# EtherealEngine/Universal-Volumetric

Hardware: AMD Instinct MI355X
Metric: frames/s encode, 100k-vert mesh + 2048^2 texture (higher is better)
Workload: dtype u8/int32 (f32 only in the quantiser)

## Files before the change

universal-volumetric_amd/csrc/geo_conn.hpp:

```cpp
__global__ void __launch_bounds__(UVOL_BLOCK) k_face_time(GeoJob *jobs) {
  JOB_OR_RETURN;
  const uint32_t i = blockIdx.x * UVOL_BLOCK + threadIdx.x;
  if (i < (uint32_t)J.nsym) { const int c = J.proc[i]; J.face_time[c / 3] = (int32_t)i; J.tstart[J.nsym - 1 - (int)i] = code_of_corner(c); }
  if (i < (uint32_t)J.ninit) { const int c = J.initc[i]; J.face_time[c / 3] = -(int32_t)i - 2; J.tstart[J.nsym + (int)i] = code_of_corner(c); }
}
__device__ __forceinline__ int att_vertex(const GeoJob &J, int slot, int c);
__device__ __forceinline__ int rec_vertex_field(const GeoJob &J, int t, int c, int r8) {
  if (r8 == 2) { const uint32_t *q = reinterpret_cast<const uint32_t *>(J.rec[1 + t]) + 4 * (size_t)(c / 3); return (int)((uint32_t)((((uint64_t)q[1] << 32) | q[0]) >> (21 * (c % 3))) & 0x1fffffu); }
  const size_t code = (size_t)code_of_corner(c);
  return r8 ? (int)((uint32_t)J.rec[1 + t][2 * code] & 0x1fffffu) : J.rec[1 + t][4 * code];
}
__global__ void __launch_bounds__(UVOL_BLOCK) k_v2d(GeoJob *jobs, int r8) {
  GeoJob &J = jobs[blockIdx.y];
  const int t = blockIdx.z;
  const uint32_t i = blockIdx.x * UVOL_BLOCK + threadIdx.x;
  const bool live = J.status == 0 && !(t > 0 && (t - 1 >= J.nad || !J.interior_seams[t - 1]));
  if (blockIdx.x * UVOL_BLOCK >= (live ? J.ne[t] : 0u)) return;
  int lo0 = 0x7fffffff, hi0 = -0x7fffffff - 1, lo1 = 0x7fffffff, hi1 = -0x7fffffff - 1;
  int iu = -1;
  if (J.qpos) for (int k = 0; k < J.nad; k++) if (J.att_kind[k] == 0 && (J.interior_seams[k] ? t == 1 + k : t == 0)) iu = k;
  if (i < J.ne[t]) {
    const int c = J.order[t][i];
    int vid, pid = 0;
    if (!J.qpos) vid = rec_vertex_field(J, t, c, r8) >> 1;
// ... 32 lines not shown
__global__ void __launch_bounds__(UVOL_BLOCK) k_eb_event_flags(GeoJob *jobs) {
  JOB_OR_RETURN_UNIFORM;
  const uint32_t i = blockIdx.x * UVOL_BLOCK + threadIdx.x;
  uint32_t n = 0;
  if (i < J.nf) { int a[2], b[2]; n = i < (uint32_t)J.nsym ? (uint32_t)eb_events_of(J, i, a, b) : 0u; J.evcnt[i] = (uint8_t)n; }
  const uint32_t tot = block_sum(n);
  if (threadIdx.x == 0 && blockIdx.x < uvol_blocks_dev(J.nf)) J.bsum2[blockIdx.x] = tot;
}
__global__ void __launch_bounds__(UVOL_BLOCK) k_eb_event_compact(GeoJob *jobs) {
  GeoJob &J = jobs[blockIdx.y];
  const uint32_t i = blockIdx.x * UVOL_BLOCK + threadIdx.x;
  if (J.status == 0 && blockIdx.x != 0 && blockIdx.x < uvol_blocks_dev(J.nf) && J.bsum2[blockIdx.x + 1] == J.bsum2[blockIdx.x]) return;
  const bool live = J.status == 0 && i < J.nf;
  uint32_t v = live ? J.evcnt[i] : 0, tot;
  const uint32_t pos = block_excl_scan(v, &tot) + ((J.status == 0 && blockIdx.x <= uvol_blocks_dev(J.nf)) ? J.bsum2[blockIdx.x] : 0);
  if (live && v) {
    int a[2], b[2]; const int n = eb_events_of(J, i, a, b);
    if (pos + (uint32_t)n > J.evcap) J.status = GEO_E_WS_OVERFLOW;
    else for (int k = 0; k < n; k++) { J.ev_src[pos + k] = (int)i; J.ev_spl[pos + k] = a[k]; J.ev_edge[pos + k] = (uint8_t)b[k]; }
  }
  if (blockIdx.x == 0 && threadIdx.x == 0 && J.status == 0) J.nev = (int)J.bsum2[uvol_blocks_dev(J.nf)];
}

__global__ void __launch_bounds__(UVOL_BLOCK) k_valence_init(GeoJob *jobs) {
  JOB_OR_RETURN;
  const uint32_t t = blockIdx.x * UVOL_BLOCK + threadIdx.x, stride = gridDim.x * UVOL_BLOCK;
  { const uint32_t n4 = J.nc / 4;
    const uint4 *src = reinterpret_cast<const uint4 *>(geo_vt(J)); uint4 *dst = reinterpret_cast<uint4 *>(J.c2vm);
    for (uint32_t q = t; q < n4; q += stride) dst[q] = src[q];
    for (uint32_t c = 4 * n4 + t; c < J.nc; c += stride) J.c2vm[c] = geo_vt(J)[c]; }
  const uint32_t nv0 = J.nverts_t[0] < J.ecap ? J.nverts_t[0] : J.ecap;
  for (uint32_t v = t; v < nv0; v += stride) J.vval[v] = J.ring_d[v];
}
__global__ void __launch_bounds__(64) k_eb_valence(GeoJob *jobs) {
  GeoJob &J = jobs[blockIdx.x];
  UVOL_SERIAL_PRIO();
  const uint32_t lane = threadIdx.x;
  const bool ok = J.status == 0;
  const int nsym = ok ? J.nsym : 0, nc = (int)J.nc;
  const int32_t *opp = J.opp, *proc = J.proc, *ftime = J.face_time; const uint8_t *symb = J.symb;
  int32_t *vval = J.vval, *c2vm = J.c2vm;
  const int nv0 = ok ? (int)J.nverts_t[0] : 0;
  (void)nc;
  int nvval = nv0;
  for (int base = 0; base < nsym; base += 64) {
    const int mi = base + (int)lane;
    int c_ = 0, s_ = 0, va_ = 0, vn_ = 0, vp_ = 0;
    if (mi < nsym) { c_ = proc[mi]; s_ = symb[mi]; va_ = c2vm[c_]; vn_ = c2vm[g_nxt(c_)]; vp_ = c2vm[g_prv(c_)]; }
    const int cnt = nsym - base < 64 ? nsym - base : 64;
    const uint32_t dpk = s_ == 0 ? 0x14u : (s_ == 5 ? 0x25u : (s_ == 3 ? 0x19u : 0x2au));
    int start = 0;
    while (start < cnt) {
      const unsigned long long smask = __ballot((int)lane >= start && (int)lane < cnt && s_ == 1);
      const int e = smask ? (int)(__ffsll((long long)smask) - 1) : cnt;
      if (e > start) {
        const bool act = (int)lane >= start && (int)lane < e;
        const int v_start = act ? UVOL_ALOAD(&vval[vn_]) : 0;
        int acc = 0;
        for (int k = start; k + 1 < e; k++) {
          const int ka = (int)UVOL_READLANE(va_, k), kn = (int)UVOL_READLANE(vn_, k), kp = (int)UVOL_READLANE(vp_, k);
          const uint32_t kd = UVOL_READLANE(dpk, k);
          const int hit = (vn_ == ka ? (int)(kd & 3u) : 0) + (vn_ == kn ? (int)((kd >> 2) & 3u) : 0) + (vn_ == kp ? (int)(kd >> 4) : 0);
          acc += (int)lane > k ? hit : 0;
        }
        if (act) {
          const int av = v_start - acc;
          if (mi > 0) { const int cv = av < 2 ? 2 : (av > 7 ? 7 : av); J.ctx_of[mi] = (uint8_t)(cv - 2); }
          if (dpk & 3u) UVOL_AADD(&vval[va_], -(int)(dpk & 3u));
          UVOL_AADD(&vval[vn_], -(int)((dpk >> 2) & 3u));
          UVOL_AADD(&vval[vp_], -(int)(dpk >> 4));
        }
        UVOL_WAVE_FENCE();
        UVOL_WAVE_SYNC();
      }
      if (e < cnt) {
        const int i = base + e;
        const int lc = (int)UVOL_READLANE(c_, e);
        const int ia = (int)UVOL_READLANE(va_, e), in_ = (int)UVOL_READLANE(vn_, e), ip = (int)UVOL_READLANE(vp_, e);
        if (lane == 0) {
          const int nx = g_nxt(lc), pv = g_prv(lc);
          const int val_n = UVOL_ALOAD(&vval[in_]), val_p = UVOL_ALOAD(&vval[ip]);
          UVOL_ASTORE(&vval[in_], val_n - 1); UVOL_ASTORE(&vval[ip], val_p - 1);
          int nleft = 0, a = opp[pv];
          while (a >= 0) { if (ftime[a / 3] <= i) break; nleft++; a = opp[g_nxt(a)]; }
          UVOL_ASTORE(&vval[ia], nleft + 1);
          const int newv = nvval; int nright = 0; a = opp[nx];
          while (a >= 0) { if (ftime[a / 3] <= i) break; nright++; c2vm[g_nxt(a)] = newv; a = opp[g_prv(a)]; }
          UVOL_ASTORE(&vval[nvval], nright + 1);
          if (i > 0) { const int cv = val_n < 2 ? 2 : (val_n > 7 ? 7 : val_n); J.ctx_of[i] = (uint8_t)(cv - 2); }
        }
        nvval++;
        UVOL_WAVE_FENCE();
        UVOL_WAVE_SYNC();
        if (mi < nsym && (int)lane > e) { va_ = c2vm[c_]; vn_ = c2vm[g_nxt(c_)]; vp_ = c2vm[g_prv(c_)]; }
      }
      start = e + 1;
    }
  }
}

__global__ void __launch_bounds__(64) k_eb_ctx(GeoJob *jobs) {
  GeoJob &J = jobs[blockIdx.x];
  UVOL_SERIAL_PRIO();
  const uint32_t lane = threadIdx.x;
  const int nsym = J.status == 0 ? J.nsym : 0;
  uint32_t cnt[6] = {0, 0, 0, 0, 0, 0};
  for (int base = 1; base < nsym; base += 64) {
    const int i = base + (int)lane;
    const int cx = i < nsym ? J.ctx_of[i] : 7;
    for (int c = 0; c < 6; c++) cnt[c] += (uint32_t)__popcll(__ballot(cx == c));
  }
  uint32_t base_c[6]; { uint32_t o = 0; for (int c = 0; c < 6; c++) { base_c[c] = o; o += cnt[c]; } }
  uint32_t *all = J.ctx_all;
  const unsigned long long lt = lane == 0 ? 0ull : (~0ull >> (64 - lane));
  for (int base = 1; base < nsym; base += 64) {
    const int i = base + (int)lane;
    const bool in = i < nsym;
    const int cx = in ? J.ctx_of[i] : 7;
    const int ps = in ? J.symb[i - 1] : 0;
    const uint32_t id = ps == 0 ? 0u : (ps == 1 ? 1u : (ps == 3 ? 2u : (ps == 5 ? 3u : 4u)));
    for (int c = 0; c < 6; c++) {
      const unsigned long long m = __ballot(in && cx == c);
      if (in && cx == c) all[base_c[c] + (uint32_t)__popcll(m & lt)] = id;
      base_c[c] += (uint32_t)__popcll(m);
    }
  }
  if (lane == 0 && J.status == 0) for (int c = 0; c < 6; c++) { J.ctx_n[c] = cnt[c]; J.rs[c].n = cnt[c]; J.ctx_sym[c] = all + (base_c[c] - cnt[c]); J.rs[c].syms = J.ctx_sym[c]; }
}

__device__ __forceinline__ bool fseam_bit(const GeoJob &J, int slot, int c) { return (J.fseam[c / 3] >> (3 * slot + c % 3)) & 1u; }
__device__ __forceinline__ int st_opp(const GeoJob &J, int slot, int c) { if (c < 0) return GEO_INV; if (slot >= 0 && fseam_bit(J, slot, c)) return GEO_INV; return J.opp[c]; }
__device__ __forceinline__ int st_swl(const GeoJob &J, int slot, int c) { const int o = st_opp(J, slot, g_nxt(c)); return o < 0 ? GEO_INV : g_nxt(o); }
__device__ __forceinline__ int st_swr(const GeoJob &J, int slot, int c) { const int o = st_opp(J, slot, g_prv(c)); return o < 0 ? GEO_INV : g_prv(o); }
__device__ __forceinline__ bool vseam_bit(const GeoJob &J, int slot, uint32_t v) { return (J.vseam[slot][v >> 5] >> (v & 31)) & 1u; }
__device__ __forceinline__ int att_vertex(const GeoJob &J, int slot, int c) {
  const int v = geo_vt(J)[c];
  return (J.interior_seams[slot] && vseam_bit(J, slot, (uint32_t)v)) ? J.avert[slot][c] : v;
}
__global__ void __launch_bounds__(UVOL_BLOCK) k_seams(GeoJob *jobs) {
  JOB_OR_RETURN;
  const uint32_t f = blockIdx.x * UVOL_BLOCK + threadIdx.x;
  if (f >= J.nf) return;
  const uvol_s3 o3 = *reinterpret_cast<const uvol_s3 *>(J.opp + 3 * (size_t)f);
  const int opp_[3] = { o3.x, o3.y, o3.z };
  uint32_t bits = 0;
  for (int i = 0; i < J.nad; i++) {
    const int32_t *A = J.att_kind[i] == 0 ? J.cu : J.cn;
    const uvol_s3 a3 = *reinterpret_cast<const uvol_s3 *>(A + 3 * (size_t)f);
    const int a[3] = { a3.x, a3.y, a3.z };
    bool any = false;
    for (int k = 0; k < 3; k++) {
      uint32_t sm = 1;
      if (opp_[k] >= 0) {
        const int oo = opp_[k], fo = 3 * (oo / 3), jo = oo - fo;
        const uvol_s3 b3 = *reinterpret_cast<const uvol_s3 *>(A + fo);
        const int b[3] = { b3.x, b3.y, b3.z };
        sm = (a[(k + 1) % 3] != b[(jo + 2) % 3] || a[(k + 2) % 3] != b[(jo + 1) % 3]) ? 1u : 0u;
        if (sm) {
          any = true;
          const uint32_t va = (uint32_t)geo_vt(J)[3 * f + (k + 1) % 3], vb = (uint32_t)geo_vt(J)[3 * f + (k + 2) % 3];
// ... 94 lines not shown
```

universal-volumetric_amd/csrc/geo_walk_simt.hpp:

```cpp
#define S_REC(code, vi, rc, lc)                                                                                         \
  do {                                                                                                                  \
    if (R8) { const uvol_u2 q_ = *(UVOL_G(const uvol_u2))(rec + 2 * (size_t)(code)); rec8_dec(q_.x, q_.y, vi, rc, lc); }  \
    else { const uvol_i4 q_ = *(UVOL_G(const uvol_i4))(rec + 4 * (size_t)(code)); vi = q_.x; rc = q_.y; lc = q_.z; }      \
  } while (0)
#define S_FLAG(code) (rec[(R8 ? 2 : 4) * (size_t)((code) | 3)])
#define S_PRE(code, a, b, c, fl)                                                                                        \
  do {                                                                                                                  \
    if (R8) { const uvol_u2 q_ = *(UVOL_G(const uvol_u2))(rec + 2 * (size_t)(code)); a = q_.x; b = q_.y; c = 0; }          \
    else { const uvol_i4 q_ = *(UVOL_G(const uvol_i4))(rec + 4 * (size_t)(code)); a = (uint32_t)q_.x; b = (uint32_t)q_.y; c = (uint32_t)q_.z; } \
    fl = S_FLAG(code);                                                                                                  \
  } while (0)
#define S_TAKE(a, b, c, vi, rc, lc) do { if (R8) rec8_dec(a, b, vi, rc, lc); else { vi = (int)(a); rc = (int)(b); lc = (int)(c); } } while (0)

template <bool R8>
__device__ inline void eb_walk_simt(GeoJob &J) {
  const int nf = (int)J.nf;
  UVOL_G(uint32_t) rec = UVOL_TO_G(uint32_t, reinterpret_cast<uint32_t *>(J.rec[0]));
  UVOL_G(uint32_t) vbits = UVOL_TO_G(uint32_t, reinterpret_cast<uint32_t *>(J.vvis));
  UVOL_G(int32_t) proc = UVOL_TO_G(int32_t, J.proc); UVOL_G(int32_t) stack = UVOL_TO_G(int32_t, J.stack); UVOL_G(int32_t) initc = UVOL_TO_G(int32_t, J.initc);
  UVOL_G(uint8_t) symb = UVOL_TO_G(uint8_t, J.symb); UVOL_G(uint8_t) start_bits = UVOL_TO_G(uint8_t, J.start_bits);
  const bool rl = J.relabel != 0; UVOL_G(const int32_t) s_of_o = UVOL_TO_G(const int32_t, J.s_of_o);
  int nproc = 0, ninit = 0, nstart = 0, nsplit = 0;
  int fo = 0, sp = 0, x = -1, vi = 0, rcn = -1, lcn = -1;
  for (;;) {
// ... 412 lines not shown
      const uint32_t unf = (uint32_t)nf;
      const uint32_t rf = ((uint32_t)rcc >> 2) < unf ? ((uint32_t)rcc >> 2) : unf, lf = ((uint32_t)lcc >> 2) < unf ? ((uint32_t)lcc >> 2) : unf;
      f16_mark<FD>(rec, fc, q);
      const uvol_u4 qr = f16_load(rec, (int)rf), ql = f16_load(rec, (int)lf);
      const uint32_t v = vic >> 1;
      const uint32_t vw = vbits[v >> 5];
      const int top2 = pend_s[pend >= 2 ? pend - 2 : 0];
      vbits[v >> 5] = vw | (1u << (v & 31));
      const uint32_t vvis = (vw >> (v & 31)) & 1u;
      order[n_ord] = 3 * fc + (x & 3);
      n_ord += (int)(vvis ^ 1u);
      nvis += run ? 1 : 0;
      const uint32_t rvis = f16_seen<FD>(qr) ? 1u : 0u, lvis = f16_seen<FD>(ql) ? 1u : 0u;
      const bool ccase = ((vvis | vic) & 1u) == 0;
      const uint32_t k = ccase ? 0u : 1u + rvis + 2u * lvis;
      pend_s[pend] = lcc;
      const bool fork = k == 1u;
      if (!run) { pend--; top = top2; }
      if (fork) { pend++; top = lcc; if (pend > (int)stcap) { J.status = GEO_E_WS_OVERFLOW; done = true; } }
      if (k == 4u) { x = -1; q.x = q.z = 0; q.y = q.w = 0x80000000u; }
      else {
        const bool go_l = k == 2u;
        x = go_l ? lcc : rcc;
        q.x = go_l ? ql.x : qr.x; q.y = go_l ? ql.y : qr.y; q.z = go_l ? ql.z : qr.z; q.w = go_l ? ql.w : qr.w;
        f16_dec(q, x & 3, vi, rc, lc);
      }
    }
  }
  if (live && J.status == 0) {
    J.ne[t] = (uint32_t)n_ord;
    if (t == 0 && J.nverts != 0xffffffffu && (uint32_t)n_ord != J.nverts) J.status = -11;
  }
}
__global__ void __launch_bounds__(64) k_traverse_wave_f16(GeoJob *jobs, int n, int W, int t0, int base_hi) {
  const int t = t0 + (int)blockIdx.y;
  if (t == 0 && base_hi) traverse_wave_f16<3>(jobs, n, W, t); else traverse_wave_f16<1>(jobs, n, W, t);
}
```

universal-volumetric_amd/csrc/geom_encode.hip:

```cpp
#include <chrono>
#include <thread>
#include "uvol_common.hpp"
#include "geom_device.hpp"
#include "uvol_ws.hpp"
#include <algorithm>
#include <map>

#define JOB_OR_RETURN GeoJob &J = jobs[blockIdx.y]; if (J.status != 0) return
#define JOB_OR_RETURN_UNIFORM GeoJob &J = jobs[blockIdx.y]; { __shared__ int job_st_; if (threadIdx.x == 0) job_st_ = J.status; __syncthreads(); if (job_st_ != 0) return; }

#include "geo_scan.hpp"
#include "geo_dedup.hpp"
#include "geo_faces.hpp"
#include "geo_corner_table.hpp"
#include "geo_walk_lds.hpp"
#include "geo_conn.hpp"
#include "geo_traverse_lds.hpp"
#include "geo_walk_simt.hpp"
#include "geo_attr.hpp"
#include "geo_matseam.hpp"
#include "geo_seq.hpp"
#include "geo_entropy.hpp"
#include "geo_layout.hpp"
struct WsItem { size_t slot, bytes; int first, last; size_t off; };
struct WsPlan {
  std::vector<uint64_t> key; std::vector<size_t> offs; size_t total = 0, zero = 0;
};
struct WsPlanCache { std::map<std::vector<uint64_t>, WsPlan> plans; };
struct GeoUp { UvolUpSlot *slot = nullptr; std::vector<size_t> off; };
struct GeoLane {
  GeoUp up;
  hipStream_t stream = nullptr, aux = nullptr; bool own_stream = false;
  bool own_aux = false;
  hipEvent_t ev_walk = nullptr, ev_val = nullptr, ev_fe = nullptr;
  uvol_devbuf slab;
  uvol_devbuf inputs;
  uvol_devbuf jobs;
  uvol_devbuf outs;
  std::vector<GeoJob> hjobs;
  uint8_t *pinned = nullptr; size_t pinned_cap = 0;
  uint32_t *counts = nullptr;
  bool busy = false, on_device = false, full = false;
  std::vector<uvol_mesh> meshes; std::vector<uint8_t *> outp; std::vector<size_t> caps;
  std::vector<const uint8_t *> mats; int frame0 = 0;
  size_t *out_lens = nullptr; int *status = nullptr; int n = 0, n_conc = 0;
  bool late_join = false;
  uint8_t *ext_out = nullptr; size_t ext_cap = 0; size_t *ext_offs = nullptr; hipStream_t producer = nullptr; hipEvent_t ev_prod = nullptr;
  std::chrono::steady_clock::time_point t_enter; double t_prep = 0, t_enq = 0;
};
struct GeoState {
  std::vector<GeoLane *> lanes; int next_lane = 0;
  hipStream_t aux = nullptr;
  int lanes_cap = 1 << 20;
  hipEvent_t walk_last = nullptr;
  hipEvent_t fe_last = nullptr;
  int deferred_rc = UVOL_OK;
  WsPlanCache plan; std::vector<WsItem> items;
  size_t max_lds = 64 * 1024;
  int num_cu = 256;
  bool blocking_call = false;
  bool compact_ok = true;
};
static void geo_lane_free(GeoLane *L) {
  if (L->aux) { (void)hipStreamSynchronize(L->aux); if (L->own_aux) (void)hipStreamDestroy(L->aux); }
  if (L->own_stream && L->stream) { (void)hipStreamSynchronize(L->stream); (void)hipStreamDestroy(L->stream); }
  for (uvol_devbuf *b : { &L->slab, &L->inputs, &L->jobs, &L->outs }) if (b->p) (void)hipFree(b->p);
  if (L->pinned) (void)hipHostFree(L->pinned);
  for (hipEvent_t e : { L->ev_walk, L->ev_val, L->ev_fe, L->ev_prod }) if (e) (void)hipEventDestroy(e);
  if (L->counts) (void)hipFree(L->counts);
  delete L;
}
static inline const UvolRingShape &geo_ring() {
  static const UvolRingShape v = [] {
    const char *l = getenv("UVOL_GEO_LANES"), *g = getenv("UVOL_GEO_GROUPS"), *a = getenv("UVOL_GEO_AUX");
    const int lf = l ? std::max(1, atoi(l)) : 0, gf = g ? std::max(1, atoi(g)) : 0;
    const int af = !a ? -1 : (strcmp(a, "shared") == 0 ? 1 : (strcmp(a, "lane") == 0 ? 0 : -1));
    const UvolRingShape s = uvol_ring_shape(uvol_hw_queues(), lf, gf, af);
    if (uvol_debug()) fprintf(stderr, "[uvol] geometry ring: %d hardware queues -> %d lanes x %d groups per call, %s auxiliary stream\n", uvol_hw_queues(), s.lanes, s.groups, s.shared_aux ? "one shared" : "per-lane");
    return s; }();
// ... 277 lines not shown
  const size_t n16 = (size_t)J.dd_cap[blockIdx.z] / 4;
  for (size_t i = (size_t)blockIdx.x * UVOL_BLOCK + threadIdx.x; i < n16; i += (size_t)gridDim.x * UVOL_BLOCK) p[i] = make_uint4(0, 0, 0, 0);
  if (blockIdx.x == 0 && threadIdx.x == 0) for (uint32_t i = (uint32_t)n16 * 4; i < J.dd_cap[blockIdx.z]; i++) J.dd_tab[blockIdx.z][i] = 0;
}

struct WalkPlan { int simt_w; size_t lds; int vcw; };
static inline int geo_relabel_mode() { static const int v = [] { const char *e = getenv("UVOL_RELABEL"); return !e ? 2 : (*e == '0' ? 0 : (*e == '1' ? 1 : 2)); }(); return v; }
static inline bool geo_relabel_on() { return geo_relabel_mode() != 0; }
static inline int geo_walk_pf() { static const int v = [] { const char *e = getenv("UVOL_WALK_PF"); return (e && *e == '0') ? 0 : 1; }(); return v; }
static inline int geo_simt_env() { static const int w = [] { const char *e = getenv("UVOL_SIMT_W"); int v = e ? atoi(e) : 0; return v < 0 ? 0 : (v > 64 ? 64 : v); }(); return w; }
static WalkPlan walk_plan(const GeoState *G, uint32_t max_nfi, uint32_t max_vals, size_t n_walkers, bool vertex_bits_global = false) {
  WalkPlan P{0, 0, 0};
  const size_t walk_fw = ((size_t)max_nfi + 31) / 32;
  const size_t lds_cu = 150 * 1024 , fw_bytes = walk_fw * 4 + (WALK_STG_DWORDS + WALK_PUB_DWORDS) * 4 + 16 ;
  const size_t v_min_bytes = std::min<size_t>((((size_t)max_vals + max_vals / 16 + 31) / 32 + 2) * 4, ((3 * (size_t)max_nfi + 31) / 32) * 4);
  static const int walk_force = [] { const char *e = getenv("UVOL_WALK_FORCE"); return !e ? 0 : (!strcmp(e, "vglobal") ? 1 : (!strcmp(e, "global") ? 2 : 0)); }();
  const bool vglobal = walk_force == 1 || vertex_bits_global;
  size_t per_cu = lds_cu / (fw_bytes + (vglobal ? 4 : v_min_bytes)); if (per_cu < 1) per_cu = 1;
  const size_t slot = (lds_cu / per_cu) & ~(size_t)1023;
  const size_t walk_vcw = vglobal ? 1 : (slot > fw_bytes + v_min_bytes ? (slot - fw_bytes) / 4 : v_min_bytes / 4);
  P.lds = (((walk_fw + walk_vcw + 3) & ~(size_t)3) + WALK_STG_DWORDS + WALK_PUB_DWORDS) * 4; P.vcw = (int)walk_vcw;
  const bool lds_fits = P.lds <= G->max_lds;
  if (geo_simt_env() > 0) P.simt_w = geo_simt_env();
  else if (walk_force == 2 || !lds_fits) P.simt_w = 1;
  else if (walk_force == 0 && n_walkers > per_cu * (size_t)G->num_cu) P.simt_w = n_walkers >= 1024 ? 16 : 4;
  return P;
}
static inline bool geo_rec8(uint32_t max_nfi, uint64_t max_ids) {
  static const bool force16 = [] { const char *e = getenv("UVOL_REC16"); return e && *e == '1'; }();
  return !force16 && 4ull * max_nfi < (1ull << 20) && max_ids < (1ull << 20);
}
bool geo_records8(uint32_t max_nfi) { return geo_rec8(max_nfi, 3ull * max_nfi); }
static inline bool geo_rec_face_off() { static const bool v = [] { const char *e = getenv("UVOL_REC_FACE"); return e && *e == '0'; }(); return v; }
static void launch_traversals(uvol_ctx *ctx, GeoJob *dj, int n, const WalkPlan &P, int r8, int base_hi = 0) {
  const unsigned N = (unsigned)n;
  if (P.simt_w) {
    const unsigned W = (unsigned)P.simt_w, nb = (3 * N + W - 1) / W;
    static const bool lane_form = [] { const char *e = getenv("UVOL_TRAV_FORM"); return e && !strcmp(e, "lane"); }();
    static const int wave_w = [] { const char *e = getenv("UVOL_TRAV_W"); const int v = e ? atoi(e) : 0; return v < 0 ? 0 : (v > 64 ? 64 : v); }();
    if (r8 == 2 && !lane_form) { const unsigned Ww = wave_w ? (unsigned)wave_w : W; LAUNCH(k_traverse_wave_f16, dim3((N + Ww - 1) / Ww, 3), dim3(64), dj, n, (int)Ww, 0, base_hi); }
    else if (r8 == 2) LAUNCH(k_traverse_simt_f16, dim3(nb), dim3(64), dj, n, (int)W, 0, 3);
    else if (r8) LAUNCH((k_traverse_simt<true>), dim3(nb), dim3(64), dj, n, (int)W); else LAUNCH((k_traverse_simt<false>), dim3(nb), dim3(64), dj, n, (int)W);
  }
  else if (r8) LAUNCH_SM((k_traverse<true>), dim3(3, N), dim3(128), P.lds, dj, P.vcw, geo_walk_pf() ? 2 : 0);
  else LAUNCH_SM((k_traverse<false>), dim3(3, N), dim3(128), P.lds, dj, P.vcw, geo_walk_pf() ? 2 : 0);
}
int geo_run_traversals(uvol_ctx *ctx, GeoJob *dj, int n, uint32_t max_nfi, uint32_t max_vals) {
  GeoState *G = ctx->geo;
  const unsigned N = (unsigned)n, bf = uvol_blocks(max_nfi), bc = uvol_blocks((size_t)3 * max_nfi);
  WalkPlan P = walk_plan(G, max_nfi, max_vals, (size_t)3 * N);
  const int r8 = geo_records8(max_nfi) ? ((P.simt_w && !geo_rec_face_off()) ? 2 : 1) : 0;
  if (P.simt_w > 1 && geo_simt_env() == 0) P.simt_w = r8 == 2 ? 4 : 1;
  for (int w = 1; w <= 3; w++) LAUNCH(k_pack_faces, dim3(bf, N), dim3(UVOL_BLOCK), dj, w, r8);
  launch_traversals(ctx, dj, n, P, r8);
  LAUNCH(k_v2d, dim3(bc, N, 3), dim3(UVOL_BLOCK), dj, r8);
  return UVOL_OK;
}

extern "C" size_t uvol_mesh_bound_mat(const uvol_mesh *m) { return m ? uvol_mesh_bound(m) + 4096 + 8 * (size_t)m->n_faces : 0; }
extern "C" size_t uvol_mesh_workspace(const uvol_ctx *ctx, const uvol_mesh *m) {
  if (!ctx || !m || !m->n_faces) return 0;
  GeoJob J{}; J.compact = 1;
  J.relabel = geo_relabel_mode(); J.n_pos = m->n_pos; J.nf_in = m->n_faces; J.n_uv = (m->uv && m->idx_uv) ? m->n_uv : 0; J.n_nrm = (m->nrm && m->idx_nrm) ? m->n_nrm : 0;
  J.qp = ctx->prm.q_position_attr; J.qt = ctx->prm.q_texture_attr; J.qn = ctx->prm.q_normal_attr;
  WsPlanCache P; std::vector<WsItem> items;
  const int fmt = geo_rec8(m->n_faces, geo_ecap(J.n_pos, J.n_uv, J.n_nrm, J.nf_in, false)) ? 2 : 0;
  const size_t big = layout_job(J, nullptr, false, fmt, fmt, P, items).total;
  WsPlanCache P1; std::vector<WsItem> items1; GeoJob J1 = J; J1.compact = 0;
  const int fmt1 = fmt ? 1 : 0;
  const size_t small = layout_job(J1, nullptr, false, fmt1, fmt1, P1, items1).total;
  return std::max(big, small) + 32768 + 8 * (size_t)m->n_faces + (sizeof(GeoJob) - GEO_JOB_MAT_BYTES);
}
static int geo_encode_sequential(uvol_ctx *ctx, GeoJob *dj, int n, bool full, uint32_t max_nfi, uint32_t max_vals, uint32_t max_ecap, uint64_t algo_in) {
// ... 87 lines not shown
  static const int face_alias = [] { const char *e = getenv("UVOL_FACE_ALIAS"); return (e && *e == '0') ? 0 : 1; }();
  const bool can_probe = (geo_relabel_on() && !seq) || std::max(n, n_conc) >= 256;
  bool compact = seq || (compact_env && face_alias && !full && can_probe && G->compact_ok);
  int rc;
  bool uploaded = false;
  const bool pre_up = !on_device && L.up.slot != nullptr;
  auto shape = [&](GeoJob &J, const uvol_mesh &m, int i, bool late) {
    J.compact = compact ? 1 : 0;
    J.n_pos = m.n_pos; J.nf_in = m.n_faces; J.relabel = seq ? 0 : geo_relabel_mode(); J.seq = seq ? 1 : 0; J.late_join = late ? 1 : 0;
    J.has_uv = (m.uv && m.idx_uv && m.n_uv) ? 1 : 0; J.has_nrm = (m.nrm && m.idx_nrm && m.n_nrm) ? 1 : 0;
    J.n_uv = J.has_uv ? m.n_uv : 0; J.n_nrm = J.has_nrm ? m.n_nrm : 0;
    J.has_mat = (mats && mats[i]) ? 1 : 0;
    J.ms.on = (J.has_mat && mseam) ? 1 : 0;
    J.qp = prm.q_position_attr; J.qt = prm.q_texture_attr; J.qn = prm.q_normal_attr;
  };
#ifndef HIPEMU
  auto ring_fits_late = [&]() -> bool {
    size_t ws = 0;
    for (int i = 0; i < n; i++) {
      const uvol_mesh &m = meshes[i]; if (!m.pos || !m.idx_pos || m.n_pos == 0 || m.n_faces == 0 || m.n_faces > (1u << 26)) return false;
      GeoJob J{}; shape(J, m, i, true);
      ws += layout_job(J, nullptr, full, fmt0, fmtT, G->plan, G->items).total;
    }
    const int ring = n_conc > n ? std::max(1, std::min(G->lanes_cap, geo_lanes_wanted(on_device))) : 1;
    std::vector<size_t> caps; bool self = false;
    for (int k = 0; k < ring; k++) { const GeoLane *o = k < (int)G->lanes.size() ? G->lanes[k] : nullptr; self = self || o == &L; caps.push_back(o ? o->slab.cap : 0); }
    if (!self) caps.push_back(L.slab.cap);
    size_t free_b = 0, total_b = 0;
    if (hipMemGetInfo(&free_b, &total_b) != hipSuccess) { (void)hipGetLastError(); return false; }
    return uvol_ws_ring_fits(ws, caps, free_b, total_b);
  };
  if (late_env < 0 && !late_small && !seq) late_join = ring_fits_late();
#endif
  L.late_join = late_join;
  auto lay = [&]() -> int {
  L.hjobs.assign((size_t)n, GeoJob{});
  ws_total = 0; in_total = 0; out_total = 0; max_ecap = 0; he_nb_max = 0; ms_nb_max = 1; he_part_all = true; algo_in = 0;
  for (int i = 0; i < n; i++) {
    const uvol_mesh &m = meshes[i]; GeoJob &J = L.hjobs[i];
    if (!m.pos || !m.idx_pos || m.n_pos == 0 || m.n_faces == 0 || m.n_faces > (1u << 26)) { ctx->set_error("mesh %d: empty or invalid", i); return UVOL_E_INVALID; }
    shape(J, m, i, late_join);
    J.mat_lo = 0xffffffffu; J.mat_hi = 0;
    J.nad = J.has_uv + J.has_nrm;
    { int k = 0; if (J.has_uv) J.att_kind[k++] = 0; if (J.has_nrm) J.att_kind[k++] = 1; for (; k < 2; k++) J.att_kind[k] = -1; }
    const WsPlan &wp = layout_job(J, nullptr, full, fmt0, fmtT, G->plan, G->items);
    ws_off[i] = ws_total; ws_total += wp.total; zero_sz[i] = wp.zero;
    const size_t in_sz = ((size_t)m.n_pos * 12 + 255) / 256 * 256 + ((size_t)J.n_uv * 8 + 255) / 256 * 256 + ((size_t)J.n_nrm * 12 + 255) / 256 * 256 +
                         (size_t)(1 + J.has_uv + J.has_nrm) * (((size_t)m.n_faces * 12 + 255) / 256 * 256) + (J.has_mat ? ((size_t)m.n_faces + 255) / 256 * 256 : 0);
    in_off[i] = in_total; in_total += (on_device || pre_up) ? 0 : in_sz;
    const size_t oc = full ? caps[i] : std::min<size_t>(caps[i], 32768 + 8 * (size_t)m.n_faces);
    out_total += (oc + 255) & ~(size_t)255; J.out_cap = (uint32_t)std::min<size_t>(caps[i], 0xffffffffu);
    max_vals = std::max(max_vals, std::max(m.n_pos, std::max(J.n_uv, J.n_nrm))); max_ecap = std::max(max_ecap, J.ecap);
    he_nb_max = std::max(he_nb_max, J.he_nb); he_part_all = he_part_all && J.he_vpb != 0;
    if (J.relabel && !J.compact) ms_nb_max = std::max(ms_nb_max, std::max(J.ms_nb[0], ((J.n_pos ? J.n_pos - 1 : 0) >> J.ms_sh[1]) + 1));
    algo_in += (uint64_t)m.n_pos * 12 + (uint64_t)J.n_uv * 8 + (uint64_t)J.n_nrm * 12 + (uint64_t)(1 + J.has_uv + J.has_nrm) * m.n_faces * 12;
  }
  if ((rc = uvol_ensure(ctx, L.slab, ws_total))) {
    (void)hipGetLastError();
    for (GeoLane *o : G->lanes) if (o != &L && o->busy) { const int r = geo_complete(ctx, *o); if (r != UVOL_OK && G->deferred_rc == UVOL_OK) G->deferred_rc = r; }
    for (GeoLane *o : G->lanes) if (o != &L && !o->busy) for (uvol_devbuf *b : { &o->slab, &o->inputs, &o->outs }) if (b->p) { (void)hipStreamSynchronize(o->stream); (void)hipFree(b->p); b->p = nullptr; b->cap = 0; }
    G->lanes_cap = std::max(1, std::min(G->lanes_cap, (int)G->lanes.size()) - 1);
    if ((rc = uvol_ensure(ctx, L.slab, ws_total))) return rc;
  }
  if ((rc = uvol_ensure(ctx, L.jobs, sizeof(GeoJob) * (size_t)n))) return rc;
  if (!L.ext_out && (rc = uvol_ensure(ctx, L.outs, out_total))) return rc;
  if (!on_device && !pre_up && (rc = uvol_ensure(ctx, L.inputs, in_total))) return rc;
  std::vector<UvolUpItem> ups; if (!on_device && !pre_up) ups.reserve((size_t)n * 6);
// ... 156 lines not shown
    } else {
      LAUNCH(k_he_count, dim3(bci, N), dim3(UVOL_BLOCK), dj);
      LAUNCH(k_he_scan, dim3(1, N), dim3(UVOL_BLOCK), dj);
      LAUNCH(k_he_fill, dim3(bci, N), dim3(UVOL_BLOCK), dj);
    }
    LAUNCH(k_edge_match, dim3(bci, N), dim3(UVOL_BLOCK), dj);
    LAUNCH(k_vert0, dim3(bv, N), dim3(UVOL_BLOCK), dj);
    LAUNCH(k_vert_fill, dim3(bc, N), dim3(UVOL_BLOCK), dj);
  }
  }
  UVOL_HIP_CHECK(ctx, hipEventRecord(L.ev_fe, ctx->stream)); G->fe_last = L.ev_fe;
  static const int w_walk_env = [] { const char *e = getenv("UVOL_SIMT_W_WALK"); const int v = e ? atoi(e) : 0; return v < 0 ? 0 : (v > 64 ? 64 : v); }();
  static const int w_trav_env = [] { const char *e = getenv("UVOL_SIMT_W_TRAV"); const int v = e ? atoi(e) : 0; return v < 0 ? 0 : (v > 64 ? 64 : v); }();
  if (w_walk_env && wp_walk.simt_w) wp_walk.simt_w = w_walk_env;
  {
    if (!fe_sliced) LAUNCH(k_pack0, dim3(bf, N), dim3(UVOL_BLOCK), dj, fmt0);
    uvol_ctx::Scope sc(ctx, "geo.k4_eb_walk", (uint64_t)n * 32 * max_nfi);
    if (wp_walk.simt_w) {
      const unsigned W = (unsigned)wp_walk.simt_w, nb = (N + W - 1) / W;
      if (fmt0 == 2) LAUNCH(k_eb_walk_simt_f16, dim3(nb), dim3(64), dj, n, (int)W);
      else if (r8) LAUNCH((k_eb_walk_simt<true>), dim3(nb), dim3(64), dj, n, (int)W); else LAUNCH((k_eb_walk_simt<false>), dim3(nb), dim3(64), dj, n, (int)W);
    }
    else if (r8) LAUNCH_SM((k_eb_walk<true>), dim3(N), dim3(128), wp_walk.lds, dj, wp_walk.vcw, geo_walk_pf());
    else LAUNCH_SM((k_eb_walk<false>), dim3(N), dim3(128), wp_walk.lds, dj, wp_walk.vcw, geo_walk_pf());
    LAUNCH(k_face_time, dim3(bf, N), dim3(UVOL_BLOCK), dj);
  }
  {
    LAUNCH(k_eb_event_flags, dim3(bf, N), dim3(UVOL_BLOCK), dj);
    LAUNCH(k_scan_sums, dim3(1, N), dim3(UVOL_BLOCK), dj, (int)SCAN_EVENTS);
    LAUNCH(k_eb_event_compact, dim3(bf, N), dim3(UVOL_BLOCK), dj);
    LAUNCH(k_valence_init, dim3(bc, N), dim3(UVOL_BLOCK), dj);
  }
  UVOL_HIP_CHECK(ctx, hipEventRecord(L.ev_walk, ctx->stream)); G->walk_last = L.ev_walk;
  UVOL_HIP_CHECK(ctx, hipStreamWaitEvent(L.aux, L.ev_walk, 0));
  {
    { uvol_ctx::Scope sc(ctx, "geo.k4_eb_valence", 0, L.aux); LAUNCH_ON(L.aux, k_eb_valence, dim3(N), dim3(64), dj); }
    LAUNCH_ON(L.aux, k_eb_ctx, dim3(N), dim3(64), dj);
  }
  UVOL_HIP_CHECK(ctx, hipEventRecord(L.ev_val, L.aux));
  {
    uvol_ctx::Scope sc(ctx, "geo.k4b_seams", 0);
    LAUNCH(k_seams, dim3(bf, N), dim3(UVOL_BLOCK), dj);
    LAUNCH(k_sb_count, dim3(bf, N), dim3(UVOL_BLOCK), dj);
    LAUNCH(k_scan_sums, dim3(1, N), dim3(UVOL_BLOCK), dj, (int)SCAN_ELIG);
    LAUNCH(k_sb_write, dim3(bf, N), dim3(UVOL_BLOCK), dj);
    LAUNCH(k_aseg_a, dim3(bci, N, 2), dim3(UVOL_BLOCK), dj);
    LAUNCH(k_aseg_b, dim3(bci, N, 2), dim3(UVOL_BLOCK), dj);
  }
  if (!late_join) UVOL_HIP_CHECK(ctx, hipStreamWaitEvent(ctx->stream, L.ev_val, 0));
  {
    if (base_shared) LAUNCH(k_pack_tabs, dim3(bf, N, 2), dim3(UVOL_BLOCK), dj, fmtT, 2); else LAUNCH(k_pack_tabs, dim3(bf, N, 3), dim3(UVOL_BLOCK), dj, fmtT, 1);
    uvol_ctx::Scope sc(ctx, "geo.k5_traverse", (uint64_t)n * 32 * max_nfi * 3);
    if (wp_trav.simt_w > 1 && !lockstep && geo_simt_env() == 0) wp_trav.simt_w = fmtT == 2 ? ((G->blocking_call && 3u * NC <= 2048u) ? 1 : ((G->blocking_call && 3u * NC <= 4096u) ? 2 : 4)) : 1;
    if (w_trav_env && wp_trav.simt_w) wp_trav.simt_w = w_trav_env;
    launch_traversals(ctx, dj, n, wp_trav, fmtT, base_shared ? 1 : 0);
  }
  if (late_join) UVOL_HIP_CHECK(ctx, hipStreamWaitEvent(ctx->stream, L.ev_val, 0));
  { uvol_ctx::Scope sc(ctx, "geo.k5b_v2d", 0); LAUNCH(k_v2d, dim3(be, N, 3), dim3(UVOL_BLOCK), dj, fmtT); }
  {
    uvol_ctx::Scope sc(ctx, "geo.k6_predict", 0);
    if (any_mat) { LAUNCH(k_mat_vert, dim3(bc, N), dim3(UVOL_BLOCK), dj, 0); LAUNCH(k_mat_vert, dim3(bc, N), dim3(UVOL_BLOCK), dj, 1); }
    if (mat_pass) {
      uvol_ctx::Scope sm(ctx, "geo.k6b_mat_seams", 0);
      LAUNCH(k_ms_flags, dim3(bf, N), dim3(UVOL_BLOCK), dj);
      LAUNCH(k_ms_sb_count, dim3(bf, N), dim3(UVOL_BLOCK), dj);
      LAUNCH(k_scan_sums, dim3(1, N), dim3(UVOL_BLOCK), dj, (int)SCAN_ELIG);
      LAUNCH(k_ms_sb_write, dim3(bf, N), dim3(UVOL_BLOCK), dj);
      LAUNCH(k_ms_aseg, dim3(bc, N), dim3(UVOL_BLOCK), dj, 0);
      LAUNCH(k_ms_aseg, dim3(bc, N), dim3(UVOL_BLOCK), dj, 1);
      LAUNCH(k_ms_pack, dim3(bf, N), dim3(UVOL_BLOCK), dj);
      LAUNCH(k_ms_traverse, dim3(N), dim3(64), dj);
      LAUNCH(k_ms_v2d, dim3(be, N), dim3(UVOL_BLOCK), dj);
      LAUNCH(k_ms_pred, dim3(be, N), dim3(UVOL_BLOCK), dj);
    }
    LAUNCH(k_stream_setup, dim3(N), dim3(64), dj);
    LAUNCH(k_pred_pos, dim3(be, N), dim3(UVOL_BLOCK), dj);
    LAUNCH(k_pred_uv, dim3(be, N), dim3(UVOL_BLOCK), dj);
    LAUNCH(k_scan_blocks, dim3(be, N), dim3(UVOL_BLOCK), dj, (int)SCAN_ORI);
    LAUNCH(k_scan_sums, dim3(1, N), dim3(UVOL_BLOCK), dj, (int)SCAN_ORI);
    LAUNCH(k_ori_compact, dim3(be, N), dim3(UVOL_BLOCK), dj);
    LAUNCH(k_ori_bits, dim3(be, N), dim3(UVOL_BLOCK), dj);
    LAUNCH(k_face_normals, dim3(bf, N), dim3(UVOL_BLOCK), dj);
    LAUNCH(k_pred_nrm, dim3(be, N), dim3(UVOL_BLOCK), dj);
    if (any_mat) LAUNCH(k_pred_mat, dim3(be, N), dim3(UVOL_BLOCK), dj);
  }
  {
    uvol_ctx::Scope sc0(ctx, "geo.k7_hist_tables", 0);
    const unsigned NS = any_mat ? GEO_NSTREAM : GEO_NSTREAM - 1;
    LAUNCH(k_hist, dim3(uvol_blocks((size_t)9 * max_nfi, 16 * UVOL_BLOCK), NS, N), dim3(UVOL_BLOCK), dj);
    LAUNCH(k_rans_tables, dim3(NS, N), dim3(64), dj);
// ... 62 lines not shown
    int st = J.status == 0 ? UVOL_OK : (J.status == UVOL_E_NOSPACE ? UVOL_E_NOSPACE : UVOL_E_ENCODE);
    out_lens[i] = J.out_len;
    if (L.ext_offs) L.ext_offs[i] = (size_t)J.out_pack_off;
    if (st == UVOL_OK) { }
    else if (!full && (J.status == GEO_E_WS_OVERFLOW || J.status == GEO_E_SLAB_FULL || J.status == GEO_E_DD_OVERFLOW)) { retry.push_back(i); st = UVOL_OK; }
    else if (J.status == GEO_E_MAT_SEAM) { st = UVOL_E_UNSUPPORTED; ctx->set_error("mesh %d: two materials meet at a shared vertex (interior material seam): not supported, encode the frame without materials", L.frame0 + i); worst = st; }
    else { ctx->set_error("mesh %d: encode failed (device status %d)", L.frame0 + i, J.status); worst = st; }
    if (status) status[i] = st;
  }
  if (!retry.empty()) {
    const std::vector<uvol_mesh> rm(L.meshes); const std::vector<uint8_t *> ro(L.outp); const std::vector<size_t> rcap(L.caps);
    const std::vector<const uint8_t *> rmat(L.mats); const int frame0 = L.frame0;
    uint8_t *const ext0 = L.ext_out; const size_t ext_cap0 = L.ext_cap; size_t *const offs0 = L.ext_offs; size_t tail = 0;
    if (ext0) for (int i = 0; i < n; i++) { const GeoJob &J = L.hjobs[i]; if (J.status == 0) tail = std::max<size_t>(tail, ((size_t)J.out_pack_off + J.out_len + 255) & ~(size_t)255); }
    for (int i : retry) {
      if (timing) fprintf(stderr, "[uvol-timing] mesh %d: re-encoding with worst-case workspace\n", i);
      int st1 = UVOL_OK;
      if (ext0) {
        if (tail >= ext_cap0) { if (status) status[i] = UVOL_E_NOSPACE; worst = UVOL_E_NOSPACE; out_lens[i] = 0; continue; }
        L.ext_out = ext0 + tail; L.ext_cap = ext_cap0 - tail; L.ext_offs = nullptr; L.producer = nullptr;
      }
      size_t cap1 = ext0 ? std::min<size_t>(ext_cap0 - tail, 0xffffffffu) : rcap[i];
      const uint8_t *mat1 = rmat.empty() ? nullptr : rmat[i];
      L.frame0 = frame0 + i;
      int rc1 = geo_submit(ctx, L, &rm[i], 1, 1, on_device, &ro[i], &cap1, out_lens + i, &st1, true, nullptr, mat1 ? &mat1 : nullptr);
      if (rc1 == UVOL_OK) rc1 = geo_complete(ctx, L);
      L.frame0 = frame0;
      if (ext0) { L.ext_out = ext0; L.ext_cap = ext_cap0; L.ext_offs = offs0; if (offs0) offs0[i] = tail; if (rc1 == UVOL_OK && st1 == UVOL_OK) tail = (tail + out_lens[i] + 255) & ~(size_t)255; }
      if (rc1 != UVOL_OK) return rc1;
      if (status) status[i] = st1;
      if (st1 != UVOL_OK) worst = st1;
    }
  }
  if (timing) fprintf(stderr, "[uvol-timing] geo group n=%d sizeof(GeoJob)=%zu %s join: host prepared %.1f ms, enqueued %.1f, gpu done %.1f, packed d2h %.1f, copied out %.1f (enter at %.1f)\n", n, sizeof(GeoJob), late_join ? "late" : "early", t_prep, t_enq, t_gpu, t_d2h, ms_since(t_enter),
                      std::chrono::duration<double, std::milli>(t_enter.time_since_epoch()).count());
  return status ? UVOL_OK : worst;
}

static int geo_submit(uvol_ctx *ctx, GeoLane &L, const uvol_mesh *meshes, int n, int n_conc, bool on_device,
                      uint8_t *const *outs, const size_t *caps, size_t *out_lens, int *status, bool full, GeoUp *pre, const uint8_t *const *mats) {
  if (pre) L.up = std::move(*pre); else { L.up.slot = nullptr; L.up.off.clear(); }
  if (mats) L.mats.assign(mats, mats + n); else L.mats.clear();
  L.meshes.assign(meshes, meshes + n); L.outp.assign(outs, outs + n); L.caps.assign(caps, caps + n);
  L.out_lens = out_lens; L.status = status; L.n = n; L.n_conc = n_conc; L.on_device = on_device; L.full = full;
  hipStream_t saved = ctx->stream; ctx->stream = L.stream;
  int rc = geo_shared_aux(ctx);
  if (rc == UVOL_OK) rc = geo_submit_impl(ctx, L, L.meshes.data(), n, n_conc, on_device, L.caps.data(), full);
  ctx->stream = saved;
  if (rc != UVOL_OK && L.up.slot) { (void)hipStreamSynchronize(L.stream); if (L.aux) (void)hipStreamSynchronize(L.aux); L.up.slot = nullptr; }
  L.busy = rc == UVOL_OK;
  return rc;
}
static int geo_complete(uvol_ctx *ctx, GeoLane &L) {
  if (!L.busy) return UVOL_OK;
  L.busy = false;
  hipStream_t saved = ctx->stream; ctx->stream = L.stream;
  const int rc = geo_complete_impl(ctx, L);
  ctx->stream = saved;
  return rc;
}

int geo_flush(uvol_ctx *ctx) {
  GeoState *G = ctx->geo; if (!G) return UVOL_OK;
  int rc = G->deferred_rc; G->deferred_rc = UVOL_OK;
  const int nl = (int)G->lanes.size();
  for (int k = 0; k < nl; k++) { GeoLane *L = G->lanes[(G->next_lane + k) % nl]; const int r = geo_complete(ctx, *L); if (rc == UVOL_OK) rc = r; }
  ctx->resolve_profile();
  return rc;
}

static inline int geo_lanes_wanted(bool on_device) { static const bool forced = getenv("UVOL_GEO_LANES") != nullptr; const int k = geo_ring().lanes; return (on_device || !forced) ? k : std::max(k, 4); }
static inline int geo_min_group() { static const int v = [] { const char *e = getenv("UVOL_GEO_MIN_GROUP"); const int k = e ? atoi(e) : 160; return k < 1 ? 1 : k; }(); return v; }

int geo_encode_batch_begin(uvol_ctx *ctx, const uvol_mesh *meshes, int n, bool on_device,
                           uint8_t *const *outs, const size_t *caps, size_t *out_lens, int *status, bool split, const uint8_t *const *mats, int frame0) {
  GeoState *G = ctx->geo;
  if (n <= 0) return UVOL_OK;
  { bool any = false; for (int i = 0; mats && i < n; i++) any = any || mats[i] != nullptr; if (!any) mats = nullptr; }
  const int want = std::max(1, std::min(G->lanes_cap, geo_lanes_wanted(on_device)));
  static const int split_env = [] { const char *e = getenv("UVOL_GEO_SPLIT"); return e ? atoi(e) : -1; }();
// ... 88 lines not shown
```

Measured before the change: 3304.

## Fuse edgebreaker valence/ctx replay into traversal kernel instead of aux stream

When late join and the wave-form f16 traversal are active, the serial valence and context replay kernels now run as extra blocks (a fourth grid row) of the traversal launch rather than as two kernels on a separate aux stream. This removes the cross-stream event wait, the aux-stream launches and the aux-stream setup on that path. The price is a larger traversal grid, where most blocks in the replay row exit at once, and the replay now shares the dispatch with the traversal waves. An environment variable can restore the aux-stream path.

```diff
diff --git a/universal-volumetric_amd/csrc/geo_conn.hpp b/universal-volumetric_amd/csrc/geo_conn.hpp
--- a/universal-volumetric_amd/csrc/geo_conn.hpp
+++ b/universal-volumetric_amd/csrc/geo_conn.hpp
@@ -88,9 +88,7 @@
   const uint32_t nv0 = J.nverts_t[0] < J.ecap ? J.nverts_t[0] : J.ecap;
   for (uint32_t v = t; v < nv0; v += stride) J.vval[v] = J.ring_d[v];
 }
-__global__ void __launch_bounds__(64) k_eb_valence(GeoJob *jobs) {
-  GeoJob &J = jobs[blockIdx.x];
-  UVOL_SERIAL_PRIO();
+__device__ __forceinline__ void eb_valence_frame(GeoJob &J) {
   const uint32_t lane = threadIdx.x;
   const bool ok = J.status == 0;
   const int nsym = ok ? J.nsym : 0, nc = (int)J.nc;
@@ -154,10 +152,12 @@
     }
   }
 }
-
-__global__ void __launch_bounds__(64) k_eb_ctx(GeoJob *jobs) {
-  GeoJob &J = jobs[blockIdx.x];
+__global__ void __launch_bounds__(64) k_eb_valence(GeoJob *jobs) {
   UVOL_SERIAL_PRIO();
+  eb_valence_frame(jobs[blockIdx.x]);
+}
+
+__device__ __forceinline__ void eb_ctx_frame(GeoJob &J) {
   const uint32_t lane = threadIdx.x;
   const int nsym = J.status == 0 ? J.nsym : 0;
   uint32_t cnt[6] = {0, 0, 0, 0, 0, 0};
@@ -182,6 +182,10 @@
     }
   }
   if (lane == 0 && J.status == 0) for (int c = 0; c < 6; c++) { J.ctx_n[c] = cnt[c]; J.rs[c].n = cnt[c]; J.ctx_sym[c] = all + (base_c[c] - cnt[c]); J.rs[c].syms = J.ctx_sym[c]; }
+}
+__global__ void __launch_bounds__(64) k_eb_ctx(GeoJob *jobs) {
+  UVOL_SERIAL_PRIO();
+  eb_ctx_frame(jobs[blockIdx.x]);
 }
 
 __device__ __forceinline__ bool fseam_bit(const GeoJob &J, int slot, int c) { return (J.fseam[c / 3] >> (3 * slot + c % 3)) & 1u; }
diff --git a/universal-volumetric_amd/csrc/geo_walk_simt.hpp b/universal-volumetric_amd/csrc/geo_walk_simt.hpp
--- a/universal-volumetric_amd/csrc/geo_walk_simt.hpp
+++ b/universal-volumetric_amd/csrc/geo_walk_simt.hpp
@@ -468,7 +468,18 @@
     if (t == 0 && J.nverts != 0xffffffffu && (uint32_t)n_ord != J.nverts) J.status = -11;
   }
 }
-__global__ void __launch_bounds__(64) k_traverse_wave_f16(GeoJob *jobs, int n, int W, int t0, int base_hi) {
+__device__ __attribute__((noinline)) void eb_replay_frame(GeoJob &J) {
+  UVOL_SERIAL_PRIO();
+  eb_valence_frame(J);
+  UVOL_WAVE_FENCE();
+  UVOL_WAVE_SYNC();
+  eb_ctx_frame(J);
+}
+__global__ void __launch_bounds__(64) k_traverse_wave_f16(GeoJob *jobs, int n, int W, int t0, int base_hi, int nt, int replay) {
+  if (replay) {
+    if ((int)blockIdx.y >= nt) { if ((int)blockIdx.x < n) eb_replay_frame(jobs[blockIdx.x]); return; }
+    if ((int)blockIdx.x * W >= n) return;
+  }
   const int t = t0 + (int)blockIdx.y;
   if (t == 0 && base_hi) traverse_wave_f16<3>(jobs, n, W, t); else traverse_wave_f16<1>(jobs, n, W, t);
 }
diff --git a/universal-volumetric_amd/csrc/geom_encode.hip b/universal-volumetric_amd/csrc/geom_encode.hip
--- a/universal-volumetric_amd/csrc/geom_encode.hip
+++ b/universal-volumetric_amd/csrc/geom_encode.hip
@@ -45,6 +45,7 @@
   std::vector<const uint8_t *> mats; int frame0 = 0;
   size_t *out_lens = nullptr; int *status = nullptr; int n = 0, n_conc = 0;
   bool late_join = false;
+  bool replay_fused = false; int fmt_trav = 0;
   uint8_t *ext_out = nullptr; size_t ext_cap = 0; size_t *ext_offs = nullptr; hipStream_t producer = nullptr; hipEvent_t ev_prod = nullptr;
   std::chrono::steady_clock::time_point t_enter; double t_prep = 0, t_enq = 0;
 };
@@ -388,13 +389,19 @@
 }
 bool geo_records8(uint32_t max_nfi) { return geo_rec8(max_nfi, 3ull * max_nfi); }
 static inline bool geo_rec_face_off() { static const bool v = [] { const char *e = getenv("UVOL_REC_FACE"); return e && *e == '0'; }(); return v; }
-static void launch_traversals(uvol_ctx *ctx, GeoJob *dj, int n, const WalkPlan &P, int r8, int base_hi = 0) {
+static inline bool geo_trav_lane_form() { static const bool v = [] { const char *e = getenv("UVOL_TRAV_FORM"); return e && !strcmp(e, "lane"); }(); return v; }
+static inline bool geo_trav_wave_form(const WalkPlan &P, int r8) { return P.simt_w && r8 == 2 && !geo_trav_lane_form(); }
+static inline int geo_replay_env() { static const int v = [] { const char *e = getenv("UVOL_REPLAY"); return !e ? -1 : (!strcmp(e, "aux") ? 0 : (!strcmp(e, "fused") ? 1 : -1)); }(); return v; }
+static void launch_traversals(uvol_ctx *ctx, GeoJob *dj, int n, const WalkPlan &P, int r8, int base_hi = 0, bool replay = false) {
   const unsigned N = (unsigned)n;
   if (P.simt_w) {
     const unsigned W = (unsigned)P.simt_w, nb = (3 * N + W - 1) / W;
-    static const bool lane_form = [] { const char *e = getenv("UVOL_TRAV_FORM"); return e && !strcmp(e, "lane"); }();
     static const int wave_w = [] { const char *e = getenv("UVOL_TRAV_W"); const int v = e ? atoi(e) : 0; return v < 0 ? 0 : (v > 64 ? 64 : v); }();
-    if (r8 == 2 && !lane_form) { const unsigned Ww = wave_w ? (unsigned)wave_w : W; LAUNCH(k_traverse_wave_f16, dim3((N + Ww - 1) / Ww, 3), dim3(64), dj, n, (int)Ww, 0, base_hi); }
+    if (geo_trav_wave_form(P, r8)) {
+      const unsigned Ww = wave_w ? (unsigned)wave_w : W, waves = (N + Ww - 1) / Ww;
+      if (replay) LAUNCH(k_traverse_wave_f16, dim3(std::max(waves, N), 4), dim3(64), dj, n, (int)Ww, 0, base_hi, 3, 1);
+      else LAUNCH(k_traverse_wave_f16, dim3(waves, 3), dim3(64), dj, n, (int)Ww, 0, base_hi, 3, 0);
+    }
     else if (r8 == 2) LAUNCH(k_traverse_simt_f16, dim3(nb), dim3(64), dj, n, (int)W, 0, 3);
     else if (r8) LAUNCH((k_traverse_simt<true>), dim3(nb), dim3(64), dj, n, (int)W); else LAUNCH((k_traverse_simt<false>), dim3(nb), dim3(64), dj, n, (int)W);
   }
@@ -548,7 +555,7 @@
   };
   if (late_env < 0 && !late_small && !seq) late_join = ring_fits_late();
 #endif
-  L.late_join = late_join;
+  L.late_join = late_join; L.replay_fused = false;
   auto lay = [&]() -> int {
   L.hjobs.assign((size_t)n, GeoJob{});
   ws_total = 0; in_total = 0; out_total = 0; max_ecap = 0; he_nb_max = 0; ms_nb_max = 1; he_part_all = true; algo_in = 0;
@@ -771,12 +778,17 @@
     LAUNCH(k_valence_init, dim3(bc, N), dim3(UVOL_BLOCK), dj);
   }
   UVOL_HIP_CHECK(ctx, hipEventRecord(L.ev_walk, ctx->stream)); G->walk_last = L.ev_walk;
-  UVOL_HIP_CHECK(ctx, hipStreamWaitEvent(L.aux, L.ev_walk, 0));
-  {
-    { uvol_ctx::Scope sc(ctx, "geo.k4_eb_valence", 0, L.aux); LAUNCH_ON(L.aux, k_eb_valence, dim3(N), dim3(64), dj); }
-    LAUNCH_ON(L.aux, k_eb_ctx, dim3(N), dim3(64), dj);
-  }
-  UVOL_HIP_CHECK(ctx, hipEventRecord(L.ev_val, L.aux));
+  const bool replay_fused = late_join && geo_trav_wave_form(wp_trav, fmtT) && geo_replay_env() != 0;
+  L.replay_fused = replay_fused; L.fmt_trav = fmtT;
+  if (!replay_fused) {
+    if ((rc = geo_shared_aux(ctx))) return rc;
+    UVOL_HIP_CHECK(ctx, hipStreamWaitEvent(L.aux, L.ev_walk, 0));
+    {
+      { uvol_ctx::Scope sc(ctx, "geo.k4_eb_valence", 0, L.aux); LAUNCH_ON(L.aux, k_eb_valence, dim3(N), dim3(64), dj); }
+      LAUNCH_ON(L.aux, k_eb_ctx, dim3(N), dim3(64), dj);
+    }
+    UVOL_HIP_CHECK(ctx, hipEventRecord(L.ev_val, L.aux));
+  }
   {
     uvol_ctx::Scope sc(ctx, "geo.k4b_seams", 0);
     LAUNCH(k_seams, dim3(bf, N), dim3(UVOL_BLOCK), dj);
@@ -792,9 +804,9 @@
     uvol_ctx::Scope sc(ctx, "geo.k5_traverse", (uint64_t)n * 32 * max_nfi * 3);
     if (wp_trav.simt_w > 1 && !lockstep && geo_simt_env() == 0) wp_trav.simt_w = fmtT == 2 ? ((G->blocking_call && 3u * NC <= 2048u) ? 1 : ((G->blocking_call && 3u * NC <= 4096u) ? 2 : 4)) : 1;
     if (w_trav_env && wp_trav.simt_w) wp_trav.simt_w = w_trav_env;
-    launch_traversals(ctx, dj, n, wp_trav, fmtT, base_shared ? 1 : 0);
-  }
-  if (late_join) UVOL_HIP_CHECK(ctx, hipStreamWaitEvent(ctx->stream, L.ev_val, 0));
+    launch_traversals(ctx, dj, n, wp_trav, fmtT, base_shared ? 1 : 0, replay_fused);
+  }
+  if (late_join && !replay_fused) UVOL_HIP_CHECK(ctx, hipStreamWaitEvent(ctx->stream, L.ev_val, 0));
   { uvol_ctx::Scope sc(ctx, "geo.k5b_v2d", 0); LAUNCH(k_v2d, dim3(be, N, 3), dim3(UVOL_BLOCK), dj, fmtT); }
   {
     uvol_ctx::Scope sc(ctx, "geo.k6_predict", 0);
@@ -923,7 +935,7 @@
       if (st1 != UVOL_OK) worst = st1;
     }
   }
-  if (timing) fprintf(stderr, "[uvol-timing] geo group n=%d sizeof(GeoJob)=%zu %s join: host prepared %.1f ms, enqueued %.1f, gpu done %.1f, packed d2h %.1f, copied out %.1f (enter at %.1f)\n", n, sizeof(GeoJob), late_join ? "late" : "early", t_prep, t_enq, t_gpu, t_d2h, ms_since(t_enter),
+  if (timing) fprintf(stderr, "[uvol-timing] geo group n=%d sizeof(GeoJob)=%zu %s join, %s replay, traversal records %d: host prepared %.1f ms, enqueued %.1f, gpu done %.1f, packed d2h %.1f, copied out %.1f (enter at %.1f)\n", n, sizeof(GeoJob), late_join ? "late" : "early", L.replay_fused ? "fused" : "aux", L.fmt_trav, t_prep, t_enq, t_gpu, t_d2h, ms_since(t_enter),
                       std::chrono::duration<double, std::milli>(t_enter.time_since_epoch()).count());
   return status ? UVOL_OK : worst;
 }
@@ -935,8 +947,7 @@
   L.meshes.assign(meshes, meshes + n); L.outp.assign(outs, outs + n); L.caps.assign(caps, caps + n);
   L.out_lens = out_lens; L.status = status; L.n = n; L.n_conc = n_conc; L.on_device = on_device; L.full = full;
   hipStream_t saved = ctx->stream; ctx->stream = L.stream;
-  int rc = geo_shared_aux(ctx);
-  if (rc == UVOL_OK) rc = geo_submit_impl(ctx, L, L.meshes.data(), n, n_conc, on_device, L.caps.data(), full);
+  int rc = geo_submit_impl(ctx, L, L.meshes.data(), n, n_conc, on_device, L.caps.data(), full);
   ctx->stream = saved;
   if (rc != UVOL_OK && L.up.slot) { (void)hipStreamSynchronize(L.stream); if (L.aux) (void)hipStreamSynchronize(L.aux); L.up.slot = nullptr; }
   L.busy = rc == UVOL_OK;
```

Result: faster. 3529 (median of 6 runs) (+6.8%).
